# SeoYeonnLee/Video-Chapter-Generation

Hardware: AMD Instinct MI355X
Metric: clip-windows/sec (16f×224²+128tok) train-step at 1/2/4/8 MI355X; % HBM roofline (higher is better)
Workload: dtype bf16; 1 GPU; TwoStream train step: TSM-ResNet-50 + BERT-base + ChapterHead(mlp), B=64 windows/GPU of 16x224^2 frames + 128 tokens, fused clip+AdamW; global_batch=64, seq_len=128, frames=16, resolution=224, text_fill=n_valid ~ U[L/2, L], parallelism=dp1

## Files before the change

video-chapter-generation_amd/csrc/bert.hip:

```cpp
#include "common.h"

using namespace vcg;

namespace {

__device__ __forceinline__ bool keep(uint64_t seed, uint64_t idx, float p) { return dropout_keep(seed, idx, p); }

template <typename T> __device__ __forceinline__ float bf_round(float v) { return to_f<T>(from_f<T>(v)); }

inline int grid_for(long long n, int bs = 256) {
  long long g = (n + bs - 1) / bs;
  if (g > 8192) g = 8192;
  if (g < 1) g = 1;
  return (int)g;
}

constexpr int LN_MAXE = 8;

template <typename T>
__global__ void embed_ln_fwd_kernel(const long long* __restrict__ ids, const float* __restrict__ word,
                                    const float* __restrict__ pos, const float* __restrict__ type,
                                    const float* __restrict__ gamma, const float* __restrict__ beta,
                                    T* __restrict__ out, float* __restrict__ mean_out, float* __restrict__ rstd_out,
                                    int L, int H, float eps, float p, uint64_t seed) {
// ... 399 lines not shown

template <typename T> __device__ __forceinline__ void ld4(const T* p, float (&v)[4]) {
  if constexpr (sizeof(T) == 4) {
    const float4 q = *reinterpret_cast<const float4*>(p);
    v[0] = q.x; v[1] = q.y; v[2] = q.z; v[3] = q.w;
  } else {
    const uint2 q = *reinterpret_cast<const uint2*>(p);
    v[0] = __uint_as_float(q.x << 16); v[1] = __uint_as_float(q.x & 0xffff0000u);
    v[2] = __uint_as_float(q.y << 16); v[3] = __uint_as_float(q.y & 0xffff0000u);
  }
}
template <typename T> __device__ __forceinline__ void st4(T* p, const float (&v)[4]) {
  if constexpr (sizeof(T) == 4) {
    *reinterpret_cast<float4*>(p) = make_float4(v[0], v[1], v[2], v[3]);
  } else {
    uint2 q;
    q.x = (uint32_t)f2bf(v[0]) | ((uint32_t)f2bf(v[1]) << 16);
    q.y = (uint32_t)f2bf(v[2]) | ((uint32_t)f2bf(v[3]) << 16);
    *reinterpret_cast<uint2*>(p) = q;
  }
}
__device__ __forceinline__ void ldf4(const float* p, float (&v)[4]) {
  const float4 q = *reinterpret_cast<const float4*>(p);
  v[0] = q.x; v[1] = q.y; v[2] = q.z; v[3] = q.w;
}

template <typename T, int NQ>
__global__ __launch_bounds__(256) void ln_fwd_rw_kernel(const T* __restrict__ x, const T* __restrict__ res,
                                                        const float* __restrict__ gamma, const float* __restrict__ beta,
                                                        T* __restrict__ out, float* __restrict__ mean_out,
                                                        float* __restrict__ rstd_out, int rows, float eps, float p,
                                                        uint64_t seed) {
  constexpr int H = 256 * NQ;
  const int lane = threadIdx.x & 63;
  const int row = blockIdx.x * 4 + (threadIdx.x >> 6);
  if (row >= rows) return;
  const long long rb = (long long)row * H;
  float v[NQ][4], r[NQ][4];
#pragma unroll
  for (int q = 0; q < NQ; ++q) {
    const int c = 4 * (lane + 64 * q);
    ld4<T>(x + rb + c, v[q]);
    if (res) ld4<T>(res + rb + c, r[q]);
  }
  float s = 0.f;
#pragma unroll
  for (int q = 0; q < NQ; ++q) {
    const int c = 4 * (lane + 64 * q);
#pragma unroll
    for (int i = 0; i < 4; ++i) {
      float a = v[q][i];
      if (p > 0.f) a = keep(seed, rb + c + i, p) ? a / (1.f - p) : 0.f;
      if (res) a += r[q][i];
      v[q][i] = a;
      s += a;
    }
  }
  const float mean = warp_sum(s) * (1.f / H);
  float s2 = 0.f;
#pragma unroll
  for (int q = 0; q < NQ; ++q)
#pragma unroll
    for (int i = 0; i < 4; ++i) {
      const float d = v[q][i] - mean;
      s2 += d * d;
    }
  const float rstd = rsqrtf(warp_sum(s2) * (1.f / H) + eps);
#pragma unroll
  for (int q = 0; q < NQ; ++q) {
    const int c = 4 * (lane + 64 * q);
    float g[4], b[4], o[4];
    ldf4(gamma + c, g);
    ldf4(beta + c, b);
#pragma unroll
    for (int i = 0; i < 4; ++i) o[i] = (v[q][i] - mean) * rstd * g[i] + b[i];
    st4<T>(out + rb + c, o);
  }
  if (lane == 0) {
    mean_out[row] = mean;
    rstd_out[row] = rstd;
  }
}

template <typename T, typename TD, int NQ, int NRED>
__global__ __launch_bounds__(256) void ln_bwd_rw_kernel(const TD* __restrict__ dout, const T* __restrict__ x,
                                                        const T* __restrict__ res, const float* __restrict__ gamma,
                                                        const float* __restrict__ mean_in,
                                                        const float* __restrict__ rstd_in, T* __restrict__ dx,
                                                        TD* __restrict__ dres, float* __restrict__ part, int rows,
                                                        float p, uint64_t seed) {
  constexpr int H = 256 * NQ;
  __shared__ float red[4][NRED][H];
  const int lane = threadIdx.x & 63, wave = threadIdx.x >> 6;
  float pg[NQ][4], pb[NQ][4], pd[NQ][4], gm[NQ][4];
#pragma unroll
  for (int q = 0; q < NQ; ++q) {
    ldf4(gamma + 4 * (lane + 64 * q), gm[q]);
#pragma unroll
    for (int i = 0; i < 4; ++i) pg[q][i] = pb[q][i] = pd[q][i] = 0.f;
  }
  const int stride = gridDim.x * 4;
  float nx[NQ][4] = {}, nr[NQ][4] = {}, nd[NQ][4] = {}, nmean = 0.f, nrstd = 0.f;
  auto load_row = [&](int row) {
    const long long rb = (long long)row * H;
    nmean = mean_in[row];
    nrstd = rstd_in[row];
#pragma unroll
    for (int q = 0; q < NQ; ++q) {
      const int c = 4 * (lane + 64 * q);
      ld4<T>(x + rb + c, nx[q]);
      if (res) ld4<T>(res + rb + c, nr[q]);
      ld4<TD>(dout + rb + c, nd[q]);
    }
  };
  if (blockIdx.x * 4 + wave < rows) load_row(blockIdx.x * 4 + wave);
  for (int row = blockIdx.x * 4 + wave; row < rows; row += stride) {
    const long long rb = (long long)row * H;
    const float mean = nmean, rstd = nrstd;
    float xv[NQ][4], rv[NQ][4], dv[NQ][4];
#pragma unroll
    for (int q = 0; q < NQ; ++q)
#pragma unroll
      for (int i = 0; i < 4; ++i) {
        xv[q][i] = nx[q][i];
        rv[q][i] = nr[q][i];
        dv[q][i] = nd[q][i];
      }
    if (row + stride < rows) load_row(row + stride);
    float a = 0.f, b = 0.f;
    uint32_t kb = 0xFFFFFFFFu;
#pragma unroll
    for (int q = 0; q < NQ; ++q) {
      const int c = 4 * (lane + 64 * q);
#pragma unroll
      for (int i = 0; i < 4; ++i) {
        float v = xv[q][i];
        if (p > 0.f) {
          const bool k = keep(seed, rb + c + i, p);
          kb = k ? kb : (kb & ~(1u << (4 * q + i)));
          v = k ? v / (1.f - p) : 0.f;
        }
        if (res) v += rv[q][i];
        const float xh = (v - mean) * rstd;
        const float d = dv[q][i];
        pg[q][i] += d * xh;
        pb[q][i] += d;
        const float dxh = d * gm[q][i];
        xv[q][i] = xh;
        dv[q][i] = dxh;
        a += dxh;
        b += dxh * xh;
      }
    }
    a = warp_sum(a) * (1.f / H);
    b = warp_sum(b) * (1.f / H);
#pragma unroll
    for (int q = 0; q < NQ; ++q) {
      const int c = 4 * (lane + 64 * q);
      float o[4], od[4];
#pragma unroll
      for (int i = 0; i < 4; ++i) {
        o[i] = rstd * (dv[q][i] - a - xv[q][i] * b);
        od[i] = (p > 0.f) ? (((kb >> (4 * q + i)) & 1u) ? o[i] / (1.f - p) : 0.f) : o[i];
        if (NRED > 2) pd[q][i] += bf_round<T>(od[i]);
      }
      if (dres) st4<TD>(dres + rb + c, o);
      if (dx) st4<T>(dx + rb + c, od);
    }
  }
#pragma unroll
  for (int q = 0; q < NQ; ++q)
#pragma unroll
    for (int i = 0; i < 4; ++i) {
      const int c = 4 * (lane + 64 * q) + i;
      red[wave][0][c] = pg[q][i];
      red[wave][1][c] = pb[q][i];
      if (NRED > 2) red[wave][NRED - 1][c] = pd[q][i];
    }
  __syncthreads();
  for (int i = threadIdx.x; i < NRED * H; i += 256) {
    const int r = i / H, c = i - r * H;
    part[(long long)blockIdx.x * NRED * H + i] = red[0][r][c] + red[1][r][c] + red[2][r][c] + red[3][r][c];
  }
}

template <typename T>
__global__ __launch_bounds__(256) void colsum_rw_kernel(const T* __restrict__ x, long long ld, int rows, int N,
                                                        float* __restrict__ part) {
  __shared__ float red[4][512];
  const int lane = threadIdx.x & 63, wave = threadIdx.x >> 6;
  const int c0 = blockIdx.y * 512 + 8 * lane;
  float acc[8];
#pragma unroll
  for (int i = 0; i < 8; ++i) acc[i] = 0.f;
  if (c0 < N) {
    for (int row = blockIdx.x * 4 + wave; row < rows; row += gridDim.x * 4) {
      float a[4], b[4];
      ld4<T>(x + (long long)row * ld + c0, a);
      ld4<T>(x + (long long)row * ld + c0 + 4, b);
#pragma unroll
      for (int i = 0; i < 4; ++i) {
        acc[i] += a[i];
        acc[4 + i] += b[i];
      }
    }
  }
#pragma unroll
  for (int i = 0; i < 8; ++i) red[wave][8 * lane + i] = acc[i];
  __syncthreads();
  for (int i = threadIdx.x; i < 512; i += 256) {
    const int c = blockIdx.y * 512 + i;
    if (c < N) part[(long long)blockIdx.x * N + c] = red[0][i] + red[1][i] + red[2][i] + red[3][i];
  }
}

template <typename T, int U>
__global__ __launch_bounds__(256) void colsum_tall_kernel(const T* __restrict__ x, long long ld, int rows, int N,
                                                          int cpr, float* __restrict__ part) {
  __shared__ float red[256][9];
  const int t = threadIdx.x, rpi = 256 / cpr;
  const int c = t % cpr, r0 = t / cpr;
  float acc[8];
#pragma unroll
  for (int i = 0; i < 8; ++i) acc[i] = 0.f;
  const long long step = (long long)gridDim.x * rpi;
  for (long long row = (long long)blockIdx.x * rpi + r0; row < rows; row += step * U) {
    float v[U][8];
#pragma unroll
    for (int u = 0; u < U; ++u) {
      const long long r = min(row + u * step, (long long)rows - 1);
      float a[4], b[4];
      ld4<T>(x + r * ld + 8 * c, a);
      ld4<T>(x + r * ld + 8 * c + 4, b);
#pragma unroll
      for (int i = 0; i < 4; ++i) {
        v[u][i] = a[i];
        v[u][4 + i] = b[i];
      }
    }
#pragma unroll
    for (int u = 0; u < U; ++u)
      if (row + u * step < rows) {
#pragma unroll
        for (int i = 0; i < 8; ++i) acc[i] += v[u][i];
      }
  }
#pragma unroll
  for (int i = 0; i < 8; ++i) red[t][i] = acc[i];
  __syncthreads();
  for (int o = t; o < N; o += 256) {
    const int cc = o >> 3, i = o & 7;
    float a = 0.f;
    for (int r = 0; r < rpi; ++r) a += red[r * cpr + cc][i];
    part[(long long)blockIdx.x * N + o] = a;
  }
}

__global__ __launch_bounds__(256) void colred16_kernel(const float* __restrict__ part, int nblocks, long long stride,
                                                       int N, int nout, float* out0, float* out1, float* out2,
                                                       int accumulate) {
  __shared__ double sa[3][16][16];
  const int tx = threadIdx.x & 15, ty = threadIdx.x >> 4;
  const int c = blockIdx.x * 16 + tx;
  double a[3] = {0, 0, 0};
  if (c < N) {
    for (int i = ty; i < nblocks; i += 16)
#pragma unroll
      for (int k = 0; k < 3; ++k)
        if (k < nout) a[k] += part[(long long)i * stride + (long long)k * N + c];
  }
#pragma unroll
  for (int k = 0; k < 3; ++k) sa[k][ty][tx] = a[k];
  __syncthreads();
  if (ty < 3 && ty < nout && c < N) {
    double t = 0;
#pragma unroll
    for (int j = 0; j < 16; ++j) t += sa[ty][j][tx];
    float* o = ty == 0 ? out0 : (ty == 1 ? out1 : out2);
    if (o) o[c] = (accumulate ? o[c] : 0.f) + (float)t;
  }
}

template <typename T>
__global__ void tanh_bwd_kernel(const T* __restrict__ dy, const T* __restrict__ t, T* __restrict__ dx, long long n) {
  for (long long i = blockIdx.x * (long long)blockDim.x + threadIdx.x; i < n; i += (long long)gridDim.x * blockDim.x) {
    const float tv = to_f<T>(t[i]);
    dx[i] = from_f<T>(to_f<T>(dy[i]) * (1.f - tv * tv));
  }
}

}


VCG_API int vcg_embed_ln_fwd(int dtype, const long long* ids, const float* word, const float* pos, const float* type,
                             const float* gamma, const float* beta, void* out, float* mean, float* rstd, int B, int L,
                             int H, float eps, float dropout_p, unsigned long long seed, hipStream_t s) {
  VCG_REQUIRE(H <= 256 * LN_MAXE, "hidden size too large");
  if (dtype == VCG_BF16)
    hipLaunchKernelGGL(embed_ln_fwd_kernel<bf16_t>, dim3(B * L), dim3(256), 0, s, ids, word, pos, type, gamma, beta,
                       (bf16_t*)out, mean, rstd, L, H, eps, dropout_p, (uint64_t)seed);
  else
    hipLaunchKernelGGL(embed_ln_fwd_kernel<float>, dim3(B * L), dim3(256), 0, s, ids, word, pos, type, gamma, beta,
                       (float*)out, mean, rstd, L, H, eps, dropout_p, (uint64_t)seed);
  VCG_LAUNCH_CHECK();
  return VCG_OK;
}

static int row_blocks(int rows, int* rpb) {
  int nb = rows < 512 ? rows : 512;
  if (nb < 1) nb = 1;
  *rpb = (rows + nb - 1) / nb;
  return (rows + *rpb - 1) / *rpb;
}

VCG_API long long vcg_ln_bwd_ws_bytes(int rows, int H) {
  int rpb;
  const int nb = row_blocks(rows, &rpb);
  return (long long)nb * 2 * H * 4 + (long long)rows * H * 4;
}

VCG_API int vcg_embed_ln_bwd(int dtype, const void* dout, const long long* ids, const float* word, const float* pos,
                             const float* type, const float* gamma, const float* mean, const float* rstd,
                             float* word_grad, float* pos_grad, float* type_grad, float* gamma_grad,
                             float* beta_grad, float* ws, long long ws_bytes, int B, int L, int H, float dropout_p,
                             unsigned long long seed, long long pad_idx, hipStream_t s) {
  const int rows = B * L;
  VCG_REQUIRE(ws_bytes >= vcg_ln_bwd_ws_bytes(rows, H), "workspace too small");
  VCG_REQUIRE(H <= SCAT_MAXE * 256, "hidden size > 1024 not supported by the word-grad reduction");
  if (dtype & VCG_GRAD_F32) dtype = VCG_F32;
  int rpb;
  const int nb = row_blocks(rows, &rpb);
  VCG_REQUIRE(L <= 2 * nb, "L > 2 * row blocks: the per-position sums would not fit the partial region");
  float* part = ws;
  float* de = ws + (long long)nb * 2 * H;
  if (dtype == VCG_BF16)
    hipLaunchKernelGGL(embed_ln_bwd_kernel<bf16_t>, dim3(nb), dim3(256), 0, s, (const bf16_t*)dout, ids, word, pos,
                       type, gamma, mean, rstd, de, part, L, H, rpb, rows, dropout_p, (uint64_t)seed);
  else
    hipLaunchKernelGGL(embed_ln_bwd_kernel<float>, dim3(nb), dim3(256), 0, s, (const float*)dout, ids, word, pos,
                       type, gamma, mean, rstd, de, part, L, H, rpb, rows, dropout_p, (uint64_t)seed);
  VCG_LAUNCH_CHECK();
  hipLaunchKernelGGL(colred_kernel, dim3((H + 63) / 64), dim3(256), 0, s, part, nb, (long long)2 * H, H, (long long)H,
                     gamma_grad, beta_grad, 1);
  VCG_LAUNCH_CHECK();
  if (word_grad) {
    hipLaunchKernelGGL(embed_scatter_kernel, dim3(rows), dim3(256), 0, s, de, ids, word_grad, H, (long long)rows,
                       pad_idx);
    VCG_LAUNCH_CHECK();
  }
  hipLaunchKernelGGL(embed_pos_kernel, dim3((H + 255) / 256, L), dim3(256), 0, s, de, pos_grad, part, B, L, H);
  VCG_LAUNCH_CHECK();
  if (type_grad) {
    hipLaunchKernelGGL(embed_type_kernel, dim3((H + 255) / 256), dim3(256), 0, s, part, type_grad, L, H);
    VCG_LAUNCH_CHECK();
  }
  return VCG_OK;
}

VCG_API int vcg_ln_fwd(int dtype, const void* x, const void* res, const float* gamma, const float* beta, void* out,
                       float* mean, float* rstd, int rows, int H, float eps, float dropout_p, unsigned long long seed,
                       hipStream_t s) {
  VCG_REQUIRE(H <= 256 * LN_MAXE, "hidden size too large");
  const int nq = H % 256 == 0 ? H / 256 : 0;
  if (nq >= 1 && nq <= 4 && rows > 0) {
    const dim3 g((rows + 3) / 4);
#define VCG_LNF(T, NQ)                                                                                               \
  hipLaunchKernelGGL((ln_fwd_rw_kernel<T, NQ>), g, dim3(256), 0, s, (const T*)x, (const T*)res, gamma, beta, (T*)out, \
                     mean, rstd, rows, eps, dropout_p, (uint64_t)seed)
#define VCG_LNF_T(T)                          \
  switch (nq) {                               \
    case 1: VCG_LNF(T, 1); break;             \
    case 2: VCG_LNF(T, 2); break;             \
    case 3: VCG_LNF(T, 3); break;             \
    default: VCG_LNF(T, 4); break;            \
  }
    if (dtype == VCG_BF16) { VCG_LNF_T(bf16_t) } else { VCG_LNF_T(float) }
#undef VCG_LNF_T
#undef VCG_LNF
    VCG_LAUNCH_CHECK();
    return VCG_OK;
  }
  if (dtype == VCG_BF16)
    hipLaunchKernelGGL(ln_fwd_kernel<bf16_t>, dim3(rows), dim3(256), 0, s, (const bf16_t*)x, (const bf16_t*)res, gamma,
                       beta, (bf16_t*)out, mean, rstd, H, eps, dropout_p, (uint64_t)seed);
  else
    hipLaunchKernelGGL(ln_fwd_kernel<float>, dim3(rows), dim3(256), 0, s, (const float*)x, (const float*)res, gamma,
                       beta, (float*)out, mean, rstd, H, eps, dropout_p, (uint64_t)seed);
  VCG_LAUNCH_CHECK();
  return VCG_OK;
}

VCG_API int vcg_ln_bwd(int dtype, const void* dout, const void* x, const void* res, const float* gamma,
                       const float* mean, const float* rstd, void* dx, void* dres, float* gamma_grad,
                       float* beta_grad, float* bias_grad, float* ws, long long ws_bytes, int rows, int H,
                       float dropout_p, unsigned long long seed, hipStream_t s) {
  const bool g32 = (dtype & VCG_GRAD_F32) != 0;
  dtype &= ~VCG_GRAD_F32;
  VCG_REQUIRE(!g32 || (dtype == VCG_BF16 && H % 256 == 0 && H <= 1024), "VCG_GRAD_F32: bf16 with H % 256 == 0, <= 1024");
  int rpb;
  const int nb = row_blocks(rows, &rpb);
  VCG_REQUIRE(ws_bytes >= (long long)nb * 2 * H * 4, "workspace too small");
  VCG_REQUIRE(!bias_grad || dx, "bias_grad is the column sum of dx");
  const int nq = H % 256 == 0 ? H / 256 : 0;
  const int nbr = (rows + 3) / 4 < 256 ? (rows + 3) / 4 : 256;
  if (nq >= 1 && nq <= 4 && rows > 0 && ((long long)nbr * 3 * H <= (long long)nb * 2 * H || g32)) {
    const int nred = bias_grad ? 3 : 2;
    VCG_REQUIRE((long long)nbr * nred * H * 4 <= ws_bytes, "workspace too small");
#define VCG_LNB(T, TD, NQ, NR)                                                                                     \
  hipLaunchKernelGGL((ln_bwd_rw_kernel<T, TD, NQ, NR>), dim3(nbr), dim3(256), 0, s, (const TD*)dout, (const T*)x,   \
                     (const T*)res, gamma, mean, rstd, (T*)dx, (TD*)dres, ws, rows, dropout_p, (uint64_t)seed)
#define VCG_LNB_Q(T, TD, NR)                     \
  switch (nq) {                                  \
    case 1: VCG_LNB(T, TD, 1, NR); break;        \
    case 2: VCG_LNB(T, TD, 2, NR); break;        \
    case 3: VCG_LNB(T, TD, 3, NR); break;        \
    default: VCG_LNB(T, TD, 4, NR); break;       \
  }
    if (dtype == VCG_BF16 && g32) {
      if (nred == 3) { VCG_LNB_Q(bf16_t, float, 3) } else { VCG_LNB_Q(bf16_t, float, 2) }
    } else if (dtype == VCG_BF16) {
      if (nred == 3) { VCG_LNB_Q(bf16_t, bf16_t, 3) } else { VCG_LNB_Q(bf16_t, bf16_t, 2) }
    } else {
      if (nred == 3) { VCG_LNB_Q(float, float, 3) } else { VCG_LNB_Q(float, float, 2) }
    }
#undef VCG_LNB_Q
#undef VCG_LNB
    VCG_LAUNCH_CHECK();
    hipLaunchKernelGGL(colred16_kernel, dim3((H + 15) / 16), dim3(256), 0, s, ws, nbr, (long long)nred * H, H, nred,
                       gamma_grad, beta_grad, bias_grad, 1);
    VCG_LAUNCH_CHECK();
    return VCG_OK;
  }
  if (dtype == VCG_BF16)
    hipLaunchKernelGGL(ln_bwd_kernel<bf16_t>, dim3(nb), dim3(256), 0, s, (const bf16_t*)dout, (const bf16_t*)x,
                       (const bf16_t*)res, gamma, mean, rstd, (bf16_t*)dx, (bf16_t*)dres, ws, H, rpb, rows, dropout_p,
                       (uint64_t)seed);
  else
    hipLaunchKernelGGL(ln_bwd_kernel<float>, dim3(nb), dim3(256), 0, s, (const float*)dout, (const float*)x,
                       (const float*)res, gamma, mean, rstd, (float*)dx, (float*)dres, ws, H, rpb, rows, dropout_p,
                       (uint64_t)seed);
  VCG_LAUNCH_CHECK();
  hipLaunchKernelGGL(colred_kernel, dim3((H + 63) / 64), dim3(256), 0, s, ws, nb, (long long)2 * H, H, (long long)H,
                     gamma_grad, beta_grad, 1);
  VCG_LAUNCH_CHECK();
  if (bias_grad) {
    if (dtype == VCG_BF16)
      hipLaunchKernelGGL(colsum_part_kernel<bf16_t>, dim3(nb), dim3(256), 0, s, (const bf16_t*)dx, (long long)H,
                         rows, H, rpb, ws);
    else
      hipLaunchKernelGGL(colsum_part_kernel<float>, dim3(nb), dim3(256), 0, s, (const float*)dx, (long long)H, rows,
                         H, rpb, ws);
    VCG_LAUNCH_CHECK();
    hipLaunchKernelGGL(colred_kernel, dim3((H + 63) / 64), dim3(256), 0, s, ws, nb, (long long)H, H, 0LL, bias_grad,
                       (float*)nullptr, 1);
    VCG_LAUNCH_CHECK();
  }
  return VCG_OK;
}

constexpr int COLSUM_TALL_BLOCKS = 1024;
static bool colsum_tall(int N, long long ld, const void* x, int rows) {
  const int cpr = N / 8;
  return N % 8 == 0 && N <= 512 && (256 % cpr) == 0 && ld % 8 == 0 && ((uintptr_t)x & 15) == 0 &&
         rows >= 8 * (256 / cpr) * 64;
}

VCG_API long long vcg_colsum_ws_bytes(int rows, int N) {
  int rpb;
  const int nb = row_blocks(rows, &rpb);
  return (long long)(nb > COLSUM_TALL_BLOCKS ? nb : COLSUM_TALL_BLOCKS) * N * 4;
}

VCG_API int vcg_colsum(int dtype, const void* x, long long ld, int rows, int N, float* out, int accumulate, float* ws,
                       long long ws_bytes, hipStream_t s) {
  int rpb;
  const int nb = row_blocks(rows, &rpb);
  VCG_REQUIRE(ws_bytes >= (long long)nb * N * 4, "workspace too small");
  if (dtype == VCG_BF16 && colsum_tall(N, ld, x, rows) && ws_bytes >= (long long)COLSUM_TALL_BLOCKS * N * 4) {
    const int cpr = N / 8, rpi = 256 / cpr;
    int nbx = (int)(((long long)rows + 4LL * rpi - 1) / (4LL * rpi));
    nbx = nbx < COLSUM_TALL_BLOCKS ? nbx : COLSUM_TALL_BLOCKS;
    hipLaunchKernelGGL((colsum_tall_kernel<bf16_t, 4>), dim3(nbx), dim3(256), 0, s, (const bf16_t*)x, ld, rows, N, cpr,
                       ws);
    VCG_LAUNCH_CHECK();
    hipLaunchKernelGGL(colred16_kernel, dim3((N + 15) / 16), dim3(256), 0, s, ws, nbx, (long long)N, N, 1, out,
                       (float*)nullptr, (float*)nullptr, accumulate);
    VCG_LAUNCH_CHECK();
    return VCG_OK;
  }
  if (N % 8 == 0 && ld % 4 == 0 && ((uintptr_t)x & 15) == 0 && rows > 0) {
    int nbx = (rows + 3) / 4;
    nbx = nbx < 128 ? nbx : 128;
    if (nbx > nb) nbx = nb;
    const dim3 g(nbx, (N + 511) / 512);
    if (dtype == VCG_BF16)
      hipLaunchKernelGGL(colsum_rw_kernel<bf16_t>, g, dim3(256), 0, s, (const bf16_t*)x, ld, rows, N, ws);
    else
      hipLaunchKernelGGL(colsum_rw_kernel<float>, g, dim3(256), 0, s, (const float*)x, ld, rows, N, ws);
    VCG_LAUNCH_CHECK();
    hipLaunchKernelGGL(colred16_kernel, dim3((N + 15) / 16), dim3(256), 0, s, ws, nbx, (long long)N, N, 1, out,
                       (float*)nullptr, (float*)nullptr, accumulate);
    VCG_LAUNCH_CHECK();
    return VCG_OK;
  }
  if (dtype == VCG_BF16)
    hipLaunchKernelGGL(colsum_part_kernel<bf16_t>, dim3(nb), dim3(256), 0, s, (const bf16_t*)x, ld, rows, N, rpb, ws);
  else
    hipLaunchKernelGGL(colsum_part_kernel<float>, dim3(nb), dim3(256), 0, s, (const float*)x, ld, rows, N, rpb, ws);
  VCG_LAUNCH_CHECK();
  hipLaunchKernelGGL(colred_kernel, dim3((N + 63) / 64), dim3(256), 0, s, ws, nb, (long long)N, N, 0LL, out,
                     (float*)nullptr, accumulate);
  VCG_LAUNCH_CHECK();
  return VCG_OK;
}

VCG_API int vcg_attn_softmax_fwd(int dtype, const void* S, const long long* mask, void* P, void* Pd, int B, int nh,
                                 int L, int Lp, float scale, float dropout_p, unsigned long long seed, hipStream_t s) {
  VCG_REQUIRE(L <= 512 && Lp >= L && Lp % 2 == 0 && Lp <= 512, "L must be <= 512, Lp even");
  dim3 grid((L + 3) / 4, B * nh);
  if (dtype == VCG_BF16)
    hipLaunchKernelGGL(attn_softmax_fwd_kernel<bf16_t>, grid, dim3(256), 0, s, (const bf16_t*)S, mask, (bf16_t*)P,
                       (bf16_t*)Pd, nh, L, Lp, scale, dropout_p, (uint64_t)seed);
  else
    hipLaunchKernelGGL(attn_softmax_fwd_kernel<float>, grid, dim3(256), 0, s, (const float*)S, mask, (float*)P,
                       (float*)Pd, nh, L, Lp, scale, dropout_p, (uint64_t)seed);
  VCG_LAUNCH_CHECK();
  return VCG_OK;
}

VCG_API int vcg_attn_softmax_bwd(int dtype, const void* dPd, const void* P, void* dS, int Z, int L, int Lp, float scale,
                                 float dropout_p, unsigned long long seed, hipStream_t s) {
  VCG_REQUIRE(L <= 512 && Lp >= L && Lp % 2 == 0 && Lp <= 512, "L must be <= 512, Lp even");
  dim3 grid((L + 3) / 4, Z);
  if (dtype == VCG_BF16)
    hipLaunchKernelGGL(attn_softmax_bwd_kernel<bf16_t>, grid, dim3(256), 0, s, (const bf16_t*)dPd, (const bf16_t*)P,
                       (bf16_t*)dS, L, Lp, scale, dropout_p, (uint64_t)seed, Z);
  else
    hipLaunchKernelGGL(attn_softmax_bwd_kernel<float>, grid, dim3(256), 0, s, (const float*)dPd, (const float*)P,
                       (float*)dS, L, Lp, scale, dropout_p, (uint64_t)seed, Z);
  VCG_LAUNCH_CHECK();
  return VCG_OK;
}

VCG_API int vcg_tanh_bwd(int dtype, const void* dy, const void* t, void* dx, long long n, hipStream_t s) {
  if (dtype == VCG_BF16)
    hipLaunchKernelGGL(tanh_bwd_kernel<bf16_t>, dim3(grid_for(n)), dim3(256), 0, s, (const bf16_t*)dy,
                       (const bf16_t*)t, (bf16_t*)dx, n);
  else
    hipLaunchKernelGGL(tanh_bwd_kernel<float>, dim3(grid_for(n)), dim3(256), 0, s, (const float*)dy, (const float*)t,
                       (float*)dx, n);
  VCG_LAUNCH_CHECK();
  return VCG_OK;
}
```

video-chapter-generation_amd/csrc/bert_attn.hip:

```cpp
#include "bert_attn_host.h"

using namespace vcg;
using namespace vcg::attn;

namespace {

__global__ __launch_bounds__(256) void bert_attn_fwd_kernel(const bf16_t* __restrict__ qkv,
                                                            const long long* __restrict__ mask,
                                                            bf16_t* __restrict__ ctx, float2* __restrict__ stats,
                                                            const int* __restrict__ seq, int nh, int Lmax, int Lp,
                                                            float scale, float p, uint64_t seed) {
  __shared__ __attribute__((aligned(16))) bf16_t Ks[LT * DH];
  __shared__ __attribute__((aligned(16))) bf16_t Vt[DH * TP];
  __shared__ uint8_t kval[LT];
  const Head hd(nh, 1, seq, Lmax, Lp);
  const int L = hd.L, H = hd.H, tid = hd.tid, w = hd.w, g = hd.g, i = hd.i;
  const bf16_t* base = qkv + hd.qo;

  load_rm(base + H, hd.ld, L, Ks, tid);
  load_transpose(base + 2 * H, hd.ld, L, Vt, nullptr, tid);
  load_key_flags(kval, mask, hd.row0, L, tid);
  s16x8 qf[2][2];
  load_frags(qf, base, hd.ld, 32 * w, L, g, i);
  __syncthreads();
  if (32 * w >= L) return;

  f32x4 sacc[2][8];
  key_tiles<8>(sacc, Ks, 0, L, qf, g, i);
  const uint32_t vb = key_bits<8>(kval, 0, g);
  const float rs = p > 0.f ? 1.f / (1.f - p) : 1.f;
  s16x8 pf[2][4];
#pragma unroll
  for (int qt = 0; qt < 2; ++qt) {
    const int q = 32 * w + 16 * qt + i;
    float mx = -INFINITY;
#pragma unroll
    for (int kt = 0; kt < 8; ++kt)
#pragma unroll
      for (int r = 0; r < 4; ++r) {
        const float v = ((vb >> (4 * kt + r)) & 1u) ? sacc[qt][kt][r] * scale : -INFINITY;
        sacc[qt][kt][r] = v;
        mx = fmaxf(mx, v);
      }
    mx = fmaxf(mx, __shfl_xor(mx, 16, 64));
    mx = fmaxf(mx, __shfl_xor(mx, 32, 64));
    const bool none = mx == -INFINITY;
    float sum = 0.f;
#pragma unroll
    for (int kt = 0; kt < 8; ++kt)
#pragma unroll
      for (int r = 0; r < 4; ++r) {
        const int key = 16 * kt + 4 * g + r;
        const float v = sacc[qt][kt][r];
        const float e = none ? (key < L ? 1.f : 0.f) : (v == -INFINITY ? 0.f : __expf(v - mx));
        sacc[qt][kt][r] = e;
        sum += e;
      }
    sum += __shfl_xor(sum, 16, 64);
    sum += __shfl_xor(sum, 32, 64);
    const float inv = 1.f / sum;
    if (g == 0 && q < L) stats[hd.so + q] = make_float2(mx, inv);
    dropout_frags(pf[qt], sacc[qt], q < L, hd.drop_row(q), inv, rs, p, seed, g);
  }

  f32x4 oacc[4][2];
#pragma unroll
  for (int dt = 0; dt < 4; ++dt)
#pragma unroll
    for (int qt = 0; qt < 2; ++qt) oacc[dt][qt] = f32x4{0.f, 0.f, 0.f, 0.f};
  pv_step(oacc, Vt, pf, L, g, i);
#pragma unroll
  for (int qt = 0; qt < 2; ++qt) {
    const int q = 32 * w + 16 * qt + i;
    if (q < L) store_row64(ctx + hd.co + (long long)q * H + 4 * g, oacc, qt);
  }
}

__global__ __launch_bounds__(256) void bert_attn_bwd_kernel(const bf16_t* __restrict__ qkv,
                                                            const bf16_t* __restrict__ dctx,
                                                            const long long* __restrict__ mask,
                                                            const float2* __restrict__ stats,
                                                            bf16_t* __restrict__ dqkv, const int* __restrict__ seq,
                                                            int nh, int Lmax, int Lp, float scale, float p,
                                                            uint64_t seed) {
  __shared__ __attribute__((aligned(16))) bf16_t Qs[LT * DH];
  __shared__ __attribute__((aligned(16))) bf16_t dOs[LT * DH];
  __shared__ __attribute__((aligned(16))) bf16_t Qt[DH * TP];
  __shared__ __attribute__((aligned(16))) bf16_t dOt[DH * TP];
  __shared__ __attribute__((aligned(16))) bf16_t Kt[DH * TP];
  __shared__ __attribute__((aligned(16))) bf16_t dSm[LT * TP];
  __shared__ float2 st[LT];
  __shared__ float Dp[4 * LT];
  __shared__ uint8_t kval[LT];
  const Head hd(nh, 1, seq, Lmax, Lp);
  const int L = hd.L, H = hd.H, tid = hd.tid, w = hd.w, g = hd.g, i = hd.i;
  const long long ld = hd.ld;
  const bf16_t* base = qkv + hd.qo;
  const bf16_t* dob = dctx + hd.co;
  bf16_t* gq = dqkv + hd.qo;

  load_transpose(base, ld, L, Qt, Qs, tid);
  load_transpose(dob, H, L, dOt, dOs, tid);
  load_transpose(base + H, ld, L, Kt, nullptr, tid);
  load_key_flags(kval, mask, hd.row0, L, tid);
  if (tid < LT) st[tid] = tid < L ? stats[hd.so + tid] : make_float2(0.f, 0.f);
  s16x8 kf[2][2], vf[2][2];
  load_frags(kf, base + H, ld, 32 * w, L, g, i);
  load_frags(vf, base + 2 * H, ld, 32 * w, L, g, i);
  __syncthreads();

  const bool wkeys = 32 * w < L;
  f32x4 sacc[8][2], pacc[8][2];
  query_tiles<8>(sacc, Qs, 0, wkeys ? L : 0, kf, g, i);
  query_tiles<8>(pacc, dOs, 0, wkeys ? L : 0, vf, g, i);
  const float rs = p > 0.f ? 1.f / (1.f - p) : 1.f;
  bool kv[2];
  int keyi[2];
#pragma unroll
  for (int kt = 0; kt < 2; ++kt) {
    keyi[kt] = 32 * w + 16 * kt + i;
    kv[kt] = kval[keyi[kt]] != 0;
  }
  uint64_t keepb = 0;
#pragma unroll
  for (int qt = 0; qt < 8; ++qt)
#pragma unroll
    for (int r = 0; r < 4; ++r) {
      const int q = 16 * qt + 4 * g + r;
      const float2 mi = st[q];
      const uint64_t rowi = hd.drop_row(q);
      float part = 0.f;
#pragma unroll
      for (int kt = 0; kt < 2; ++kt) {
        const int key = keyi[kt];
        const float P = attn_prob(sacc[qt][kt][r], scale, mi, kv[kt], key < L, q < L);
        const bool keep = q < L && key < L && dropout_keep(seed, rowi + key, p);
        const float dP = keep ? pacc[qt][kt][r] * rs : 0.f;
        keepb |= keep ? (1ull << (8 * qt + 2 * r + kt)) : 0ull;
        sacc[qt][kt][r] = P;
        pacc[qt][kt][r] = dP;
        part = fmaf(P, dP, part);
      }
      part += __shfl_xor(part, 1, 64);
      part += __shfl_xor(part, 2, 64);
      part += __shfl_xor(part, 4, 64);
      part += __shfl_xor(part, 8, 64);
      if (i == 0) Dp[w * LT + q] = part;
    }
  __syncthreads();
#pragma unroll
  for (int qt = 0; qt < 8; ++qt)
#pragma unroll
    for (int r = 0; r < 4; ++r) {
      const int q = 16 * qt + 4 * g + r;
      const float D = (Dp[q] + Dp[LT + q]) + (Dp[2 * LT + q] + Dp[3 * LT + q]);
#pragma unroll
      for (int kt = 0; kt < 2; ++kt) {
        const float P = sacc[qt][kt][r];
        const float dS = scale * P * (pacc[qt][kt][r] - D);
        sacc[qt][kt][r] = ((keepb >> (8 * qt + 2 * r + kt)) & 1ull) ? P * rs : 0.f;
        pacc[qt][kt][r] = dS;
        dSm[q * TP + keyi[kt]] = f2bf(dS);
      }
    }

  f32x4 dv[4][2], dk[4][2];
#pragma unroll
  for (int dt = 0; dt < 4; ++dt)
#pragma unroll
    for (int kt = 0; kt < 2; ++kt) dv[dt][kt] = dk[dt][kt] = f32x4{0.f, 0.f, 0.f, 0.f};
#pragma unroll
  for (int s = 0; s < 4; ++s)
    if (wkeys && 32 * s < L)
      dvdk_step(dv, dk, sacc[2 * s], sacc[2 * s + 1], pacc[2 * s], pacc[2 * s + 1], dOt, Qt, 32 * s, g, i);
#pragma unroll
  for (int kt = 0; kt < 2; ++kt) {
    const int key = keyi[kt];
    if (key < L) {
      bf16_t* o = gq + (long long)key * ld + 4 * g;
      store_row64(o + H, dk, kt);
      store_row64(o + 2 * H, dv, kt);
    }
  }
  __syncthreads();

  f32x4 dq[4][2];
#pragma unroll
  for (int dt = 0; dt < 4; ++dt)
#pragma unroll
    for (int qt = 0; qt < 2; ++qt) dq[dt][qt] = f32x4{0.f, 0.f, 0.f, 0.f};
#pragma unroll
  for (int s = 0; s < 4; ++s) {
    if (32 * w >= L || 32 * s >= L) continue;
    s16x8 sbq[2];
#pragma unroll
    for (int qt = 0; qt < 2; ++qt)
      sbq[qt] = *reinterpret_cast<const s16x8*>(dSm + (32 * w + 16 * qt + i) * TP + 32 * s + 8 * g);
#pragma unroll
    for (int dt = 0; dt < 4; ++dt) {
      const s16x8 ka = *reinterpret_cast<const s16x8*>(Kt + (16 * dt + i) * TP + 32 * s + 8 * g);
#pragma unroll
      for (int qt = 0; qt < 2; ++qt) dq[dt][qt] = __builtin_amdgcn_mfma_f32_16x16x32_bf16(ka, sbq[qt], dq[dt][qt], 0, 0, 0);
    }
  }
#pragma unroll
  for (int qt = 0; qt < 2; ++qt) {
    const int q = 32 * w + 16 * qt + i;
    if (q < L) store_row64(gq + (long long)q * ld + 4 * g, dq, qt);
  }
}

int attn_check(const char* fn, const void* qkv, const void* io, const void* stats, int B, int nh, int L, int Lp,
               int* nT) {
  if (!qkv || !io || !stats || B < 0 || nh <= 0 || L < 0 || Lp < L) {
    set_error(std::string(fn) + ": invalid arguments");
    return VCG_ERR_INVALID;
  }
  if (L > LMAX) {
    set_error(std::string(fn) + ": L > 512 is not supported by the fused kernels");
    return VCG_ERR_UNSUPPORTED;
  }
  *nT = stats_tiles(L);
  if ((long long)B * nh * *nT > 0x7fffffffLL) {
    set_error(std::string(fn) + ": the tiled kernels take 128 < L <= 512");
    return VCG_ERR_UNSUPPORTED;
  }
  return VCG_OK;
}

}

VCG_API long long vcg_bert_attn_stats_bytes(int B, int nh, int L) {
  if (B < 0 || nh < 0 || L < 0) return 0;
  return stats_rows(B, nh, L) * (long long)(L <= LT ? sizeof(float2) : sizeof(float2) + sizeof(float));
}

VCG_API int vcg_bert_attn_fwd_varlen(const void* qkv, const long long* mask, const int* seq, void* ctx, void* stats,
                                     int B, int nh, int Lmax, int Lp, float scale, float dropout_p,
                                     unsigned long long seed, hipStream_t s) {
  if (B == 0 || Lmax == 0) return VCG_OK;
  int nT;
  const int rc = attn_check("vcg_bert_attn_fwd", qkv, ctx, stats, B, nh, Lmax, Lp, &nT);
  if (rc != VCG_OK) return rc;
  if (Lmax > LT)
    return bert_attn_long_fwd(qkv, mask, seq, ctx, stats, B, nh, Lmax, Lp, nT, scale, dropout_p, seed, s);
  hipLaunchKernelGGL(bert_attn_fwd_kernel, dim3(B * nh), dim3(256), 0, s, (const bf16_t*)qkv, mask, (bf16_t*)ctx,
                     (float2*)stats, seq, nh, Lmax, Lp, scale, dropout_p, (uint64_t)seed);
  VCG_CHECK_HIP(hipGetLastError());
  return VCG_OK;
}

VCG_API int vcg_bert_attn_fwd(const void* qkv, const long long* mask, void* ctx, void* stats, int B, int nh, int L,
                              int Lp, float scale, float dropout_p, unsigned long long seed, hipStream_t s) {
  return vcg_bert_attn_fwd_varlen(qkv, mask, nullptr, ctx, stats, B, nh, L, Lp, scale, dropout_p, seed, s);
}

VCG_API int vcg_bert_attn_bwd_varlen(const void* qkv, const void* dctx, const long long* mask, const int* seq,
                                     const void* stats, void* dqkv, int B, int nh, int Lmax, int Lp, float scale,
                                     float dropout_p, unsigned long long seed, hipStream_t s) {
  if (B == 0 || Lmax == 0) return VCG_OK;
  if (!dctx) {
    set_error("vcg_bert_attn_bwd: invalid arguments");
    return VCG_ERR_INVALID;
  }
  int nT;
  const int rc = attn_check("vcg_bert_attn_bwd", qkv, dqkv, stats, B, nh, Lmax, Lp, &nT);
// ... 17 lines not shown
```

video-chapter-generation_amd/csrc/bert_attn_steps.h:

```cpp
#pragma once
#include "common.h"

namespace vcg {
namespace attn {

constexpr int LT = 128;
constexpr int LMAX = 512;
constexpr int DH = 64;
constexpr int TP = 136;

__device__ __forceinline__ int swz(int row, int chunk) { return chunk ^ ((row >> 1) & 7); }

__device__ __forceinline__ uint32_t pack2(float a, float b) { return (uint32_t)f2bf(a) | ((uint32_t)f2bf(b) << 16); }

__device__ __forceinline__ uint32_t half16(const uint4& v, int j) {
  const uint32_t w = (j >> 1) == 0 ? v.x : (j >> 1) == 1 ? v.y : (j >> 1) == 2 ? v.z : v.w;
  return (j & 1) ? (w >> 16) : (w & 0xffffu);
}

__device__ __forceinline__ s16x8 frag_rm(const bf16_t* t, int row, int chunk) {
  return *reinterpret_cast<const s16x8*>(t + row * DH + 8 * swz(row, chunk));
}

__device__ __forceinline__ s16x8 frag_split(const bf16_t* t, int row, int c0) {
  const uint2 lo = *reinterpret_cast<const uint2*>(t + row * TP + c0);
  const uint2 hi = *reinterpret_cast<const uint2*>(t + row * TP + c0 + 16);
  typedef unsigned u32x4 __attribute__((ext_vector_type(4)));
  const u32x4 u = {lo.x, lo.y, hi.x, hi.y};
  return __builtin_bit_cast(s16x8, u);
}

__device__ __forceinline__ s16x8 pack8(const f32x4& a, const f32x4& b) {
  typedef unsigned u32x4 __attribute__((ext_vector_type(4)));
  const u32x4 u = {pack2(a[0], a[1]), pack2(a[2], a[3]), pack2(b[0], b[1]), pack2(b[2], b[3])};
  return __builtin_bit_cast(s16x8, u);
}

__device__ __forceinline__ uint4 ld16(const bf16_t* p, bool ok) {
  return ok ? *reinterpret_cast<const uint4*>(p) : make_uint4(0u, 0u, 0u, 0u);
}

struct Head {
  int z, tile0, row0, L, H;
  int tid, w, g, i;
  long long ld;
  long long qo, co, so;
  int Lmax, Lp;

  __device__ __forceinline__ Head(int nh, int nT, const int* seq, int Lmax_, int Lp_) : Lmax(Lmax_), Lp(Lp_) {
    z = blockIdx.x / nT;
    tile0 = LT * (blockIdx.x - z * nT);
    const int b = z / nh, h = z - b * nh;
    H = nh * DH;
    ld = 3LL * H;
    tid = threadIdx.x;
    w = tid >> 6;
    g = (tid & 63) >> 4;
    i = tid & 15;
    row0 = seq ? seq[b] : b * Lmax;
    L = seq ? seq[b + 1] - row0 : Lmax;
    qo = (long long)row0 * ld + h * DH;
    co = (long long)row0 * H + h * DH;
    so = (long long)z * (nT * LT);
  }
  __device__ __forceinline__ uint64_t drop_row(int q) const { return ((uint64_t)z * Lmax + q) * (uint64_t)Lp; }
};

__device__ __forceinline__ void load_rm(const bf16_t* src, long long ld, int nrows, bf16_t* rm, int tid) {
  for (int c = tid; c < LT * 8; c += 256) {
    const int r = c >> 3, ch = c & 7;
    *reinterpret_cast<uint4*>(rm + r * DH + 8 * swz(r, ch)) = ld16(src + (long long)r * ld + 8 * ch, r < nrows);
  }
}

__device__ __forceinline__ void load_transpose(const bf16_t* src, long long ld, int L, bf16_t* t, bf16_t* rm, int tid) {
  const int kg = tid >> 3, dc = tid & 7;
  uint4 v[4];
#pragma unroll
  for (int e = 0; e < 4; ++e) v[e] = ld16(src + (long long)(4 * kg + e) * ld + 8 * dc, 4 * kg + e < L);
  if (rm) {
#pragma unroll
    for (int e = 0; e < 4; ++e) {
      const int r = 4 * kg + e;
      *reinterpret_cast<uint4*>(rm + r * DH + 8 * swz(r, dc)) = v[e];
    }
  }
#pragma unroll
  for (int j = 0; j < 8; ++j) {
    uint2 q;
    q.x = half16(v[0], j) | (half16(v[1], j) << 16);
    q.y = half16(v[2], j) | (half16(v[3], j) << 16);
    *reinterpret_cast<uint2*>(t + (8 * dc + j) * TP + 4 * kg) = q;
  }
}

__device__ __forceinline__ void load_key_flags(uint8_t* kval, const long long* mask, long long row, int nkeys, int tid) {
  if (tid < LT) kval[tid] = tid < nkeys && (mask == nullptr || mask[row + tid] != 0);
}

__device__ __forceinline__ void load_frags(s16x8 (&f)[2][2], const bf16_t* src, long long ld, int r0, int nrows, int g,
                                           int i) {
#pragma unroll
  for (int t = 0; t < 2; ++t)
#pragma unroll
    for (int s = 0; s < 2; ++s) {
      const int r = r0 + 16 * t + i;
      f[t][s] = __builtin_bit_cast(s16x8, ld16(src + (long long)r * ld + 8 * (4 * s + g), r < nrows));
    }
}

template <int NT>
__device__ __forceinline__ void key_tiles(f32x4 (&acc)[2][NT], const bf16_t* a, int r0, int nrows,
                                          const s16x8 (&bf)[2][2], int g, int i) {
#pragma unroll
  for (int qt = 0; qt < 2; ++qt)
#pragma unroll
    for (int kt = 0; kt < NT; ++kt) acc[qt][kt] = f32x4{0.f, 0.f, 0.f, 0.f};
#pragma unroll
  for (int kt = 0; kt < NT; ++kt)
    if (r0 + 16 * kt < nrows) {
#pragma unroll
      for (int s = 0; s < 2; ++s) {
        const s16x8 af = frag_rm(a, r0 + 16 * kt + i, 4 * s + g);
#pragma unroll
        for (int qt = 0; qt < 2; ++qt) acc[qt][kt] = __builtin_amdgcn_mfma_f32_16x16x32_bf16(af, bf[qt][s], acc[qt][kt], 0, 0, 0);
      }
    }
}

template <int NT>
__device__ __forceinline__ uint32_t key_bits(const uint8_t* kval, int r0, int g) {
  uint32_t vb = 0;
#pragma unroll
  for (int kt = 0; kt < NT; ++kt)
#pragma unroll
    for (int r = 0; r < 4; ++r) vb |= kval[r0 + 16 * kt + 4 * g + r] ? (1u << (4 * kt + r)) : 0u;
  return vb;
}

__device__ __forceinline__ void dropout_frags(s16x8 (&pf)[4], const f32x4 (&e)[8], bool row, uint64_t rowi, float inv,
                                              float rs, float p, uint64_t seed, int g) {
#pragma unroll
  for (int s = 0; s < 4; ++s) {
    f32x4 a, c;
#pragma unroll
    for (int r = 0; r < 4; ++r) {
      const int k0 = 32 * s + 4 * g + r, k1 = k0 + 16;
      const float p0 = e[2 * s][r] * inv, p1 = e[2 * s + 1][r] * inv;
      a[r] = (row && dropout_keep(seed, rowi + k0, p)) ? p0 * rs : 0.f;
      c[r] = (row && dropout_keep(seed, rowi + k1, p)) ? p1 * rs : 0.f;
    }
    pf[s] = pack8(a, c);
  }
}

__device__ __forceinline__ void pv_step(f32x4 (&oacc)[4][2], const bf16_t* Vt, const s16x8 (&pf)[2][4], int nkeys, int g,
                                        int i) {
#pragma unroll
  for (int s = 0; s < 4; ++s)
    if (32 * s < nkeys) {
#pragma unroll
      for (int dt = 0; dt < 4; ++dt) {
        const s16x8 vf = frag_split(Vt, 16 * dt + i, 32 * s + 4 * g);
#pragma unroll
        for (int qt = 0; qt < 2; ++qt) oacc[dt][qt] = __builtin_amdgcn_mfma_f32_16x16x32_bf16(vf, pf[qt][s], oacc[dt][qt], 0, 0, 0);
      }
    }
}

template <int NT>
__device__ __forceinline__ void query_tiles(f32x4 (&acc)[NT][2], const bf16_t* a, int r0, int nrows,
                                            const s16x8 (&bf)[2][2], int g, int i) {
#pragma unroll
  for (int qt = 0; qt < NT; ++qt)
#pragma unroll
    for (int kt = 0; kt < 2; ++kt) acc[qt][kt] = f32x4{0.f, 0.f, 0.f, 0.f};
#pragma unroll
  for (int qt = 0; qt < NT; ++qt)
// ... 48 lines not shown
```

Baseline: 918.2 clip-windows/sec.

## Widen LN backward to 8 waves, split colred by output, alias attn-bwd LDS

The LayerNorm backward kernel is templated on waves per block and prefetch depth. It now runs 8 waves with a two-stage shared-memory reduction, and the workspace reduction kernel splits its outputs across grid.y and unrolls its loads. The attention backward kernel aliases Q/dO with dS and Qt with Kt in LDS and requests 2 blocks per CU, so K is loaded into registers early and written to LDS only after the dV/dK phase. The aim is more memory parallelism and occupancy, at the cost of extra syncs, fewer LN blocks and possible register pressure.

```diff
diff --git a/video-chapter-generation_amd/csrc/bert.hip b/video-chapter-generation_amd/csrc/bert.hip
--- a/video-chapter-generation_amd/csrc/bert.hip
+++ b/video-chapter-generation_amd/csrc/bert.hip
@@ -505,13 +505,15 @@
   }
 }
 
-template <typename T, typename TD, int NQ, int NRED>
-__global__ __launch_bounds__(256) void ln_bwd_rw_kernel(const TD* __restrict__ dout, const T* __restrict__ x,
-                                                        const T* __restrict__ res, const float* __restrict__ gamma,
-                                                        const float* __restrict__ mean_in,
-                                                        const float* __restrict__ rstd_in, T* __restrict__ dx,
-                                                        TD* __restrict__ dres, float* __restrict__ part, int rows,
-                                                        float p, uint64_t seed) {
+template <typename T, typename TD, int NQ, int NRED, int NW, int PF>
+__global__ __launch_bounds__(64 * NW) void ln_bwd_rw_kernel(const TD* __restrict__ dout, const T* __restrict__ x,
+                                                            const T* __restrict__ res,
+                                                            const float* __restrict__ gamma,
+                                                            const float* __restrict__ mean_in,
+                                                            const float* __restrict__ rstd_in, T* __restrict__ dx,
+                                                            TD* __restrict__ dres, float* __restrict__ part, int rows,
+                                                            float p, uint64_t seed) {
+  static_assert(NW == 4 || NW == 8, "4 or 8 waves");
   constexpr int H = 256 * NQ;
   __shared__ float red[4][NRED][H];
   const int lane = threadIdx.x & 63, wave = threadIdx.x >> 6;
@@ -522,86 +524,105 @@
 #pragma unroll
     for (int i = 0; i < 4; ++i) pg[q][i] = pb[q][i] = pd[q][i] = 0.f;
   }
-  const int stride = gridDim.x * 4;
-  float nx[NQ][4] = {}, nr[NQ][4] = {}, nd[NQ][4] = {}, nmean = 0.f, nrstd = 0.f;
-  auto load_row = [&](int row) {
+  const int stride = gridDim.x * NW;
+  float nx[PF][NQ][4] = {}, nr[PF][NQ][4] = {}, nd[PF][NQ][4] = {}, nmean[PF] = {}, nrstd[PF] = {};
+  auto load_row = [&](int u, int row) {
     const long long rb = (long long)row * H;
-    nmean = mean_in[row];
-    nrstd = rstd_in[row];
+    nmean[u] = mean_in[row];
+    nrstd[u] = rstd_in[row];
 #pragma unroll
     for (int q = 0; q < NQ; ++q) {
       const int c = 4 * (lane + 64 * q);
-      ld4<T>(x + rb + c, nx[q]);
-      if (res) ld4<T>(res + rb + c, nr[q]);
-      ld4<TD>(dout + rb + c, nd[q]);
+      ld4<T>(x + rb + c, nx[u][q]);
+      if (res) ld4<T>(res + rb + c, nr[u][q]);
+      ld4<TD>(dout + rb + c, nd[u][q]);
     }
   };
-  if (blockIdx.x * 4 + wave < rows) load_row(blockIdx.x * 4 + wave);
-  for (int row = blockIdx.x * 4 + wave; row < rows; row += stride) {
-    const long long rb = (long long)row * H;
-    const float mean = nmean, rstd = nrstd;
-    float xv[NQ][4], rv[NQ][4], dv[NQ][4];
+  const int row0 = blockIdx.x * NW + wave;
+#pragma unroll
+  for (int u = 0; u < PF; ++u)
+    if ((long long)row0 + (long long)u * stride < rows) load_row(u, row0 + u * stride);
+  for (long long rowp = row0; rowp < rows; rowp += (long long)PF * stride) {
+#pragma unroll
+    for (int u = 0; u < PF; ++u) {
+      const long long rowl = rowp + (long long)u * stride;
+      if (rowl >= rows) break;
+      const int row = (int)rowl;
+      const long long rb = (long long)row * H;
+      const float mean = nmean[u], rstd = nrstd[u];
+      float xv[NQ][4], rv[NQ][4], dv[NQ][4];
+#pragma unroll
+      for (int q = 0; q < NQ; ++q)
+#pragma unroll
+        for (int i = 0; i < 4; ++i) {
+          xv[q][i] = nx[u][q][i];
+          rv[q][i] = nr[u][q][i];
+          dv[q][i] = nd[u][q][i];
+        }
+      if (rowl + (long long)PF * stride < rows) load_row(u, row + PF * stride);
+      float a = 0.f, b = 0.f;
+      uint32_t kb = 0xFFFFFFFFu;
+#pragma unroll
+      for (int q = 0; q < NQ; ++q) {
+        const int c = 4 * (lane + 64 * q);
+#pragma unroll
+        for (int i = 0; i < 4; ++i) {
+          float v = xv[q][i];
+          if (p > 0.f) {
+            const bool k = keep(seed, rb + c + i, p);
+            kb = k ? kb : (kb & ~(1u << (4 * q + i)));
+            v = k ? v / (1.f - p) : 0.f;
+          }
+          if (res) v += rv[q][i];
+          const float xh = (v - mean) * rstd;
+          const float d = dv[q][i];
+          pg[q][i] += d * xh;
+          pb[q][i] += d;
+          const float dxh = d * gm[q][i];
+          xv[q][i] = xh;
+          dv[q][i] = dxh;
+          a += dxh;
+          b += dxh * xh;
+        }
+      }
+      a = warp_sum(a) * (1.f / H);
+      b = warp_sum(b) * (1.f / H);
+#pragma unroll
+      for (int q = 0; q < NQ; ++q) {
+        const int c = 4 * (lane + 64 * q);
+        float o[4], od[4];
+#pragma unroll
+        for (int i = 0; i < 4; ++i) {
+          o[i] = rstd * (dv[q][i] - a - xv[q][i] * b);
+          od[i] = (p > 0.f) ? (((kb >> (4 * q + i)) & 1u) ? o[i] / (1.f - p) : 0.f) : o[i];
+          if (NRED > 2) pd[q][i] += bf_round<T>(od[i]);
+        }
+        if (dres) st4<TD>(dres + rb + c, o);
+        if (dx) st4<T>(dx + rb + c, od);
+      }
+    }
+  }
+  auto put = [&](bool add) {
 #pragma unroll
     for (int q = 0; q < NQ; ++q)
 #pragma unroll
       for (int i = 0; i < 4; ++i) {
-        xv[q][i] = nx[q][i];
-        rv[q][i] = nr[q][i];
-        dv[q][i] = nd[q][i];
-      }
-    if (row + stride < rows) load_row(row + stride);
-    float a = 0.f, b = 0.f;
-    uint32_t kb = 0xFFFFFFFFu;
-#pragma unroll
-    for (int q = 0; q < NQ; ++q) {
-      const int c = 4 * (lane + 64 * q);
-#pragma unroll
-      for (int i = 0; i < 4; ++i) {
-        float v = xv[q][i];
-        if (p > 0.f) {
-          const bool k = keep(seed, rb + c + i, p);
-          kb = k ? kb : (kb & ~(1u << (4 * q + i)));
-          v = k ? v / (1.f - p) : 0.f;
-        }
-        if (res) v += rv[q][i];
-        const float xh = (v - mean) * rstd;
-        const float d = dv[q][i];
-        pg[q][i] += d * xh;
-        pb[q][i] += d;
-        const float dxh = d * gm[q][i];
-        xv[q][i] = xh;
-        dv[q][i] = dxh;
-        a += dxh;
-        b += dxh * xh;
-      }
-    }
-    a = warp_sum(a) * (1.f / H);
-    b = warp_sum(b) * (1.f / H);
-#pragma unroll
-    for (int q = 0; q < NQ; ++q) {
-      const int c = 4 * (lane + 64 * q);
-      float o[4], od[4];
-#pragma unroll
-      for (int i = 0; i < 4; ++i) {
-        o[i] = rstd * (dv[q][i] - a - xv[q][i] * b);
-        od[i] = (p > 0.f) ? (((kb >> (4 * q + i)) & 1u) ? o[i] / (1.f - p) : 0.f) : o[i];
-        if (NRED > 2) pd[q][i] += bf_round<T>(od[i]);
-      }
-      if (dres) st4<TD>(dres + rb + c, o);
-      if (dx) st4<T>(dx + rb + c, od);
-    }
-  }
-#pragma unroll
-  for (int q = 0; q < NQ; ++q)
-#pragma unroll
-    for (int i = 0; i < 4; ++i) {
-      const int c = 4 * (lane + 64 * q) + i;
-      red[wave][0][c] = pg[q][i];
-      red[wave][1][c] = pb[q][i];
-      if (NRED > 2) red[wave][NRED - 1][c] = pd[q][i];
-    }
+        const int c = 4 * (lane + 64 * q) + i;
+        float* r0 = &red[wave & 3][0][c];
+        float* r1 = &red[wave & 3][1][c];
+        float* r2 = &red[wave & 3][NRED - 1][c];
+        *r0 = add ? *r0 + pg[q][i] : pg[q][i];
+        *r1 = add ? *r1 + pb[q][i] : pb[q][i];
+        if (NRED > 2) *r2 = add ? *r2 + pd[q][i] : pd[q][i];
+      }
+  };
+  if (NW == 8) {
+    if (wave >= 4) put(false);
+    __syncthreads();
+  }
+  if (wave < 4) put(NW == 8);
   __syncthreads();
-  for (int i = threadIdx.x; i < NRED * H; i += 256) {
+  for (int i = threadIdx.x; i < NRED * H; i += 64 * NW) {
     const int r = i / H, c = i - r * H;
     part[(long long)blockIdx.x * NRED * H + i] = red[0][r][c] + red[1][r][c] + red[2][r][c] + red[3][r][c];
   }
@@ -679,27 +700,34 @@
   }
 }
 
+constexpr int COLRED_U = 8;
 __global__ __launch_bounds__(256) void colred16_kernel(const float* __restrict__ part, int nblocks, long long stride,
-                                                       int N, int nout, float* out0, float* out1, float* out2,
-                                                       int accumulate) {
-  __shared__ double sa[3][16][16];
+                                                       int N, float* out0, float* out1, float* out2, int accumulate) {
+  __shared__ double sa[16][16];
   const int tx = threadIdx.x & 15, ty = threadIdx.x >> 4;
-  const int c = blockIdx.x * 16 + tx;
-  double a[3] = {0, 0, 0};
+  const int c = blockIdx.x * 16 + tx, k = blockIdx.y;
+  double a = 0;
   if (c < N) {
-    for (int i = ty; i < nblocks; i += 16)
-#pragma unroll
-      for (int k = 0; k < 3; ++k)
-        if (k < nout) a[k] += part[(long long)i * stride + (long long)k * N + c];
-  }
-#pragma unroll
-  for (int k = 0; k < 3; ++k) sa[k][ty][tx] = a[k];
+    const float* src = part + (long long)k * N + c;
+    for (int i0 = ty; i0 < nblocks; i0 += 16 * COLRED_U) {
+      float v[COLRED_U];
+#pragma unroll
+      for (int u = 0; u < COLRED_U; ++u) {
+        const int i = i0 + 16 * u;
+        v[u] = i < nblocks ? src[(long long)i * stride] : 0.f;
+      }
+#pragma unroll
+      for (int u = 0; u < COLRED_U; ++u)
+        if (i0 + 16 * u < nblocks) a += v[u];
+    }
+  }
+  sa[ty][tx] = a;
   __syncthreads();
-  if (ty < 3 && ty < nout && c < N) {
+  if (ty == 0 && c < N) {
     double t = 0;
 #pragma unroll
-    for (int j = 0; j < 16; ++j) t += sa[ty][j][tx];
-    float* o = ty == 0 ? out0 : (ty == 1 ? out1 : out2);
+    for (int j = 0; j < 16; ++j) t += sa[j][tx];
+    float* o = k == 0 ? out0 : (k == 1 ? out1 : out2);
     if (o) o[c] = (accumulate ? o[c] : 0.f) + (float)t;
   }
 }
@@ -813,6 +841,8 @@
   return VCG_OK;
 }
 
+constexpr int LNB_WAVES = 8, LNB_PREFETCH = 1;
+
 VCG_API int vcg_ln_bwd(int dtype, const void* dout, const void* x, const void* res, const float* gamma,
                        const float* mean, const float* rstd, void* dx, void* dres, float* gamma_grad,
                        float* beta_grad, float* bias_grad, float* ws, long long ws_bytes, int rows, int H,
@@ -825,13 +855,14 @@
   VCG_REQUIRE(ws_bytes >= (long long)nb * 2 * H * 4, "workspace too small");
   VCG_REQUIRE(!bias_grad || dx, "bias_grad is the column sum of dx");
   const int nq = H % 256 == 0 ? H / 256 : 0;
-  const int nbr = (rows + 3) / 4 < 256 ? (rows + 3) / 4 : 256;
+  const int nbr = (rows + LNB_WAVES - 1) / LNB_WAVES < 256 ? (rows + LNB_WAVES - 1) / LNB_WAVES : 256;
   if (nq >= 1 && nq <= 4 && rows > 0 && ((long long)nbr * 3 * H <= (long long)nb * 2 * H || g32)) {
     const int nred = bias_grad ? 3 : 2;
     VCG_REQUIRE((long long)nbr * nred * H * 4 <= ws_bytes, "workspace too small");
 #define VCG_LNB(T, TD, NQ, NR)                                                                                     \
-  hipLaunchKernelGGL((ln_bwd_rw_kernel<T, TD, NQ, NR>), dim3(nbr), dim3(256), 0, s, (const TD*)dout, (const T*)x,   \
-                     (const T*)res, gamma, mean, rstd, (T*)dx, (TD*)dres, ws, rows, dropout_p, (uint64_t)seed)
+  hipLaunchKernelGGL((ln_bwd_rw_kernel<T, TD, NQ, NR, LNB_WAVES, LNB_PREFETCH>), dim3(nbr), dim3(64 * LNB_WAVES), 0, \
+                     s, (const TD*)dout, (const T*)x, (const T*)res, gamma, mean, rstd, (T*)dx, (TD*)dres, ws, rows, \
+                     dropout_p, (uint64_t)seed)
 #define VCG_LNB_Q(T, TD, NR)                     \
   switch (nq) {                                  \
     case 1: VCG_LNB(T, TD, 1, NR); break;        \
@@ -849,7 +880,7 @@
 #undef VCG_LNB_Q
 #undef VCG_LNB
     VCG_LAUNCH_CHECK();
-    hipLaunchKernelGGL(colred16_kernel, dim3((H + 15) / 16), dim3(256), 0, s, ws, nbr, (long long)nred * H, H, nred,
+    hipLaunchKernelGGL(colred16_kernel, dim3((H + 15) / 16, nred), dim3(256), 0, s, ws, nbr, (long long)nred * H, H,
                        gamma_grad, beta_grad, bias_grad, 1);
     VCG_LAUNCH_CHECK();
     return VCG_OK;
@@ -906,7 +937,7 @@
     hipLaunchKernelGGL((colsum_tall_kernel<bf16_t, 4>), dim3(nbx), dim3(256), 0, s, (const bf16_t*)x, ld, rows, N, cpr,
                        ws);
     VCG_LAUNCH_CHECK();
-    hipLaunchKernelGGL(colred16_kernel, dim3((N + 15) / 16), dim3(256), 0, s, ws, nbx, (long long)N, N, 1, out,
+    hipLaunchKernelGGL(colred16_kernel, dim3((N + 15) / 16), dim3(256), 0, s, ws, nbx, (long long)N, N, out,
                        (float*)nullptr, (float*)nullptr, accumulate);
     VCG_LAUNCH_CHECK();
     return VCG_OK;
@@ -921,7 +952,7 @@
     else
       hipLaunchKernelGGL(colsum_rw_kernel<float>, g, dim3(256), 0, s, (const float*)x, ld, rows, N, ws);
     VCG_LAUNCH_CHECK();
-    hipLaunchKernelGGL(colred16_kernel, dim3((N + 15) / 16), dim3(256), 0, s, ws, nbx, (long long)N, N, 1, out,
+    hipLaunchKernelGGL(colred16_kernel, dim3((N + 15) / 16), dim3(256), 0, s, ws, nbx, (long long)N, N, out,
                        (float*)nullptr, (float*)nullptr, accumulate);
     VCG_LAUNCH_CHECK();
     return VCG_OK;
diff --git a/video-chapter-generation_amd/csrc/bert_attn.hip b/video-chapter-generation_amd/csrc/bert_attn.hip
--- a/video-chapter-generation_amd/csrc/bert_attn.hip
+++ b/video-chapter-generation_amd/csrc/bert_attn.hip
@@ -76,19 +76,22 @@
   }
 }
 
-__global__ __launch_bounds__(256) void bert_attn_bwd_kernel(const bf16_t* __restrict__ qkv,
-                                                            const bf16_t* __restrict__ dctx,
-                                                            const long long* __restrict__ mask,
-                                                            const float2* __restrict__ stats,
-                                                            bf16_t* __restrict__ dqkv, const int* __restrict__ seq,
-                                                            int nh, int Lmax, int Lp, float scale, float p,
-                                                            uint64_t seed) {
-  __shared__ __attribute__((aligned(16))) bf16_t Qs[LT * DH];
-  __shared__ __attribute__((aligned(16))) bf16_t dOs[LT * DH];
-  __shared__ __attribute__((aligned(16))) bf16_t Qt[DH * TP];
+__global__ __launch_bounds__(256, 2) void bert_attn_bwd_kernel(const bf16_t* __restrict__ qkv,
+                                                               const bf16_t* __restrict__ dctx,
+                                                               const long long* __restrict__ mask,
+                                                               const float2* __restrict__ stats,
+                                                               bf16_t* __restrict__ dqkv, const int* __restrict__ seq,
+                                                               int nh, int Lmax, int Lp, float scale, float p,
+                                                               uint64_t seed) {
+  static_assert(2 * LT * DH <= LT * TP, "dSm covers Qs | dOs");
+  __shared__ __attribute__((aligned(16))) bf16_t QdO_dS[LT * TP];
+  __shared__ __attribute__((aligned(16))) bf16_t Qt_Kt[DH * TP];
   __shared__ __attribute__((aligned(16))) bf16_t dOt[DH * TP];
-  __shared__ __attribute__((aligned(16))) bf16_t Kt[DH * TP];
-  __shared__ __attribute__((aligned(16))) bf16_t dSm[LT * TP];
+  bf16_t* const Qs = QdO_dS;
+  bf16_t* const dOs = QdO_dS + LT * DH;
+  bf16_t* const dSm = QdO_dS;
+  bf16_t* const Qt = Qt_Kt;
+  bf16_t* const Kt = Qt_Kt;
   __shared__ float2 st[LT];
   __shared__ float Dp[4 * LT];
   __shared__ uint8_t kval[LT];
@@ -101,7 +104,6 @@
 
   load_transpose(base, ld, L, Qt, Qs, tid);
   load_transpose(dob, H, L, dOt, dOs, tid);
-  load_transpose(base + H, ld, L, Kt, nullptr, tid);
   load_key_flags(kval, mask, hd.row0, L, tid);
   if (tid < LT) st[tid] = tid < L ? stats[hd.so + tid] : make_float2(0.f, 0.f);
   s16x8 kf[2][2], vf[2][2];
@@ -169,6 +171,8 @@
   for (int dt = 0; dt < 4; ++dt)
 #pragma unroll
     for (int kt = 0; kt < 2; ++kt) dv[dt][kt] = dk[dt][kt] = f32x4{0.f, 0.f, 0.f, 0.f};
+  uint4 krows[4];
+  rows4_load(krows, base + H, ld, L, tid);
 #pragma unroll
   for (int s = 0; s < 4; ++s)
     if (wkeys && 32 * s < L)
@@ -182,6 +186,8 @@
       store_row64(o + 2 * H, dv, kt);
     }
   }
+  __syncthreads();
+  rows4_store(krows, Kt, nullptr, tid);
   __syncthreads();
 
   f32x4 dq[4][2];
diff --git a/video-chapter-generation_amd/csrc/bert_attn_steps.h b/video-chapter-generation_amd/csrc/bert_attn_steps.h
--- a/video-chapter-generation_amd/csrc/bert_attn_steps.h
+++ b/video-chapter-generation_amd/csrc/bert_attn_steps.h
@@ -73,11 +73,14 @@
   }
 }
 
-__device__ __forceinline__ void load_transpose(const bf16_t* src, long long ld, int L, bf16_t* t, bf16_t* rm, int tid) {
+__device__ __forceinline__ void rows4_load(uint4 (&v)[4], const bf16_t* src, long long ld, int L, int tid) {
   const int kg = tid >> 3, dc = tid & 7;
-  uint4 v[4];
 #pragma unroll
   for (int e = 0; e < 4; ++e) v[e] = ld16(src + (long long)(4 * kg + e) * ld + 8 * dc, 4 * kg + e < L);
+}
+
+__device__ __forceinline__ void rows4_store(const uint4 (&v)[4], bf16_t* t, bf16_t* rm, int tid) {
+  const int kg = tid >> 3, dc = tid & 7;
   if (rm) {
 #pragma unroll
     for (int e = 0; e < 4; ++e) {
@@ -94,6 +97,12 @@
   }
 }
 
+__device__ __forceinline__ void load_transpose(const bf16_t* src, long long ld, int L, bf16_t* t, bf16_t* rm, int tid) {
+  uint4 v[4];
+  rows4_load(v, src, ld, L, tid);
+  rows4_store(v, t, rm, tid);
+}
+
 __device__ __forceinline__ void load_key_flags(uint8_t* kval, const long long* mask, long long row, int nkeys, int tid) {
   if (tid < LT) kval[tid] = tid < nkeys && (mask == nullptr || mask[row + tid] != 0);
 }
```

New measurement: 917.6 clip-windows/sec. About the same (-0.1%).
